# ChuheHong/arm-spmv

Hardware: AMD Instinct MI355X
Metric: SpMV GFLOP/s + achieved HBM GB/s (% roofline), fp64 CSR, 1/2/4/8 MI355X (higher is better)
Workload: dtype f64

## Files before the change

### arm-spmv_amd/csrc/kernels_csr_panel.hip

```cpp
#include <vector>

#include <atomic>

#include "common.hpp"
#include "panel_groups.hpp"
#include "panel_settings.hpp"
#include "wave.hpp"

namespace spmv
{
namespace
{
constexpr int kPanelThreads = 1024;
constexpr int kLineDoubles  = 16;

__global__ __launch_bounds__(256) void panel_count_kernel(const int32_t* __restrict__ gstart, int W, int P,
                                                          const int32_t* __restrict__ row_ptr,
                                                          const int32_t* __restrict__ col,
                                                          int32_t* __restrict__ tile_ptr )
{
    extern __shared__ int32_t hist[];
    const int g  = blockIdx.x;
    const int r0 = gstart[g], r1 = gstart[g + 1];
    for (int i = threadIdx.x; i <= P; i += blockDim.x) hist[i] = 0;
    __syncthreads();
    const int begin = row_ptr[r0], end = row_ptr[r1];
    for (int e = begin + threadIdx.x; e < end; e += blockDim.x) atomicAdd(&hist[col[e] / W], 1);
    __syncthreads();
    if (threadIdx.x < kWave)
    {
        const int lane  = threadIdx.x;
        int       carry = 0;
        for (int base = 0; base < P; base += kWave)
        {
            const int v    = (base + lane < P) ? hist[base + lane] : 0;
            int       incl = v;
            for (int d = 1; d < kWave; d <<= 1)
            {
                const int up = bpermute(incl, max(lane - d, 0));
                if (lane >= d) incl += up;
            }
            if (base + lane < P) tile_ptr[(size_t)g * (P + 1) + base + lane] = carry + incl - v;
            carry += bpermute(incl, kWave - 1);
        }
        if (lane == 0) tile_ptr[(size_t)g * (P + 1) + P] = carry;
    }
}

__global__ __launch_bounds__(256) void panel_scatter_kernel(const int32_t* __restrict__ gstart, int W, int P,
                                                            const int32_t* __restrict__ row_ptr,
                                                            const int32_t* __restrict__ col,
                                                            const double* __restrict__ val,
                                                            const int32_t* __restrict__ tile_ptr,
                                                            int32_t* __restrict__ out_col, uint16_t* __restrict__ out_row,
                                                            double* __restrict__ out_val)
{
    extern __shared__ int32_t cursor[];
    constexpr int LPR = 8;
    const int     g   = blockIdx.x;
    const int     r0 = gstart[g], r1 = gstart[g + 1];
    for (int i = threadIdx.x; i < P; i += blockDim.x) cursor[i] = tile_ptr[(size_t)g * (P + 1) + i];
    __syncthreads();
    const int base = row_ptr[r0];
    for (int r = r0 + threadIdx.x / LPR; r < r1; r += blockDim.x / LPR)
    {
        const int end = row_ptr[r + 1];
        for (int j = row_ptr[r] + threadIdx.x % LPR; j < end; j += LPR)
        {
            const int c   = col[j];
            const int pos = base + atomicAdd(&cursor[c / W], 1);
            out_col[pos]  = c;
            out_row[pos]  = (uint16_t)(r - r0);
            out_val[pos]  = val[j];
        }
    }
}

__global__ __launch_bounds__(256) void panel_line_sort_kernel(int64_t ntiles, const int32_t* __restrict__ gstart, int W, int P,
                                                              const int32_t* __restrict__ row_ptr,
                                                              const int32_t* __restrict__ tile_ptr,
                                                              const int32_t* __restrict__ src_col,
                                                              const uint16_t* __restrict__ src_row,
                                                              const double* __restrict__ src_val,
                                                              int32_t* __restrict__ dst_col, uint16_t* __restrict__ dst_row,
                                                              double* __restrict__ dst_val)
{
    extern __shared__ int32_t bins[];
    const int nb = W / kLineDoubles;
    for (int64_t tile = blockIdx.x; tile < ntiles; tile += gridDim.x)
    {
    const int g    = (int)(tile / P);
    const int p    = (int)(tile % P);
    const int base = row_ptr[gstart[g]];
    const int t0   = base + tile_ptr[(size_t)g * (P + 1) + p];
    const int t1   = base + tile_ptr[(size_t)g * (P + 1) + p + 1];
    if (t0 == t1) continue;
    const int c0 = p * W;
    for (int i = threadIdx.x; i <= nb; i += blockDim.x) bins[i] = 0;
    __syncthreads();
    for (int e = t0 + threadIdx.x; e < t1; e += blockDim.x) atomicAdd(&bins[(src_col[e] - c0) / kLineDoubles], 1);
    __syncthreads();
    if (threadIdx.x < kWave)
    {
        const int lane  = threadIdx.x;
        int       carry = 0;
        for (int b = 0; b < nb; b += kWave)
        {
            const int v    = (b + lane < nb) ? bins[b + lane] : 0;
            int       incl = v;
            for (int d = 1; d < kWave; d <<= 1)
            {
                const int up = bpermute(incl, max(lane - d, 0));
                if (lane >= d) incl += up;
            }
            if (b + lane < nb) bins[b + lane] = carry + incl - v;
            carry += bpermute(incl, kWave - 1);
        }
    }
    __syncthreads();
    for (int e = t0 + threadIdx.x; e < t1; e += blockDim.x)
    {
        const int c   = src_col[e];
        const int pos = t0 + atomicAdd(&bins[(c - c0) / kLineDoubles], 1);
        dst_col[pos]  = c;
        dst_row[pos]  = src_row[e];
        dst_val[pos]  = src_val[e];
    }
    __syncthreads();
    }
}

using u32x2p = unsigned __attribute__((ext_vector_type(2)));

template <int UNROLL, int LAYOUT>
struct PanelBatch
{
    int      c[UNROLL];
    unsigned r[UNROLL];
    double   v[UNROLL];
    __device__ __forceinline__ void unpack(const int32_t* __restrict__ sb, int rowbits)
    {
        if constexpr (LAYOUT >= 3)
        {
#pragma unroll
            for (int u = 0; u < UNROLL; ++u)
            {
                const unsigned w = (unsigned)c[u];
                c[u]             = sb[u] + (int)(w >> rowbits);
                r[u]             = w & ((1u << rowbits) - 1u);
            }
        }
    }
    __device__ __forceinline__ void load(const int32_t* __restrict__ pcol, const uint16_t* __restrict__ prow,
                                         const double* __restrict__ pval, int e, const int32_t* __restrict__ sb = nullptr,
                                         int rowbits = 0)
    {
        load_raw(pcol, prow, pval, e);
        unpack(sb, rowbits);
    }
    __device__ __forceinline__ void load_raw(const int32_t* __restrict__ pcol, const uint16_t* __restrict__ prow,
                                             const double* __restrict__ pval, int e)
    {
        if constexpr (LAYOUT == 4 && UNROLL >= 2)
        {
            const int     t  = e & (kPanelThreads - 1);
            const size_t  p0 = (size_t)(e >> 11) * kPanelThreads + t;
            const u32x2p* w2 = reinterpret_cast<const u32x2p*>(pcol) + p0;
            const f64x2*  v2 = reinterpret_cast<const f64x2*>(pval) + p0;
#pragma unroll
            for (int u = 0; u < UNROLL / 2; ++u)
            {
                const u32x2p w = load_stream(w2 + (size_t)u * kPanelThreads);
                const f64x2  d = load_stream(v2 + (size_t)u * kPanelThreads);
                c[2 * u]       = (int)w.x;
                c[2 * u + 1]   = (int)w.y;
                v[2 * u]       = d.x;
                v[2 * u + 1]   = d.y;
            }
        }
        else if constexpr (LAYOUT == 4)
        {
            const int    t  = e & (kPanelThreads - 1), sl = e >> 10;
            const size_t at = ((size_t)(sl >> 1) << 11) + 2 * (size_t)t + (size_t)(sl & 1);
            c[0]            = load_stream(pcol + at);
            v[0]            = load_stream(pval + at);
        }
        else
        {
#pragma unroll
            for (int u = 0; u < UNROLL; ++u)
            {
                c[u] = load_stream(pcol + e + u * kPanelThreads);
                if constexpr (LAYOUT < 3) r[u] = load_stream(prow + e + u * kPanelThreads);
                v[u] = load_stream(pval + e + u * kPanelThreads);
            }
        }
    }
    __device__ __forceinline__ void apply(const double* __restrict__ x, double* acc) const
    {
        double xv[UNROLL];
        gather(x, xv);
        add(acc, xv);
    }
    __device__ __forceinline__ void gather(const double* __restrict__ x, double (&xv)[UNROLL]) const
    {
#pragma unroll
        for (int u = 0; u < UNROLL; ++u) xv[u] = x[c[u]];
    }
    __device__ __forceinline__ void add(double* acc, const double (&xv)[UNROLL]) const
    {
#pragma unroll
        for (int u = 0; u < UNROLL; ++u) atomicAdd(&acc[r[u]], v[u] * xv[u]);
    }
    __device__ static __forceinline__ void one(const int32_t* __restrict__ pcol, const uint16_t* __restrict__ prow,
                                               const double* __restrict__ pval, int e, const double* __restrict__ x,
                                               double* acc, const int32_t* __restrict__ sb = nullptr, int rowbits = 0)
    {
        PanelBatch<1, LAYOUT> b;
        b.load(pcol, prow, pval, e, sb, rowbits);
        b.apply(x, acc);
    }
};

struct PanelPacked
{
    const int32_t* sbase;
    const int32_t* soff;
    int            rowbits;
};

__global__ void panel_cut_kernel(const int32_t* __restrict__ gstart, int ngroups, const int32_t* __restrict__ row_ptr,
                                 const int32_t* __restrict__ col, int colbits, const int32_t* __restrict__ soff,
                                 int32_t* __restrict__ nslices, int32_t* __restrict__ sbase, int32_t* __restrict__ ssrc,
                                 int32_t* __restrict__ scount)
{
    const int g = blockIdx.x * blockDim.x + threadIdx.x;
    if (g >= ngroups) return;
    const int begin = row_ptr[gstart[g]], end = row_ptr[gstart[g + 1]];
    int       pos = begin, k = 0;
    while (pos < end)
    {
        const int base_line  = col[pos] / kLineDoubles;
        const int limit_line = base_line + (1 << (colbits - 4));
        const int most       = min(kPanelThreads, end - pos);
        int       take       = most;
        if (col[pos + most - 1] / kLineDoubles >= limit_line)
        {
            int lo = 1, hi = most - 1;
            while (lo < hi)
            {
                const int mid = (lo + hi + 1) / 2;
                if (col[pos + mid - 1] / kLineDoubles < limit_line)
                    lo = mid;
                else
                    hi = mid - 1;
            }
            take = lo;
        }
        if (soff)
        {
            const int idx = soff[g] + k;
            sbase[idx]    = base_line * kLineDoubles;
            ssrc[idx]     = pos;
            scount[idx]   = take;
        }
        pos += take;
        ++k;
    }
    if (!soff) nslices[g] = k;
}

__global__ __launch_bounds__(256) void panel_expand_kernel(int total, const int32_t* __restrict__ sbase,
                                                           const int32_t* __restrict__ ssrc,
                                                           const int32_t* __restrict__ scount, const int32_t* __restrict__ col,
                                                           const uint16_t* __restrict__ row, const double* __restrict__ val,
                                                           int rowbits, unsigned pad_row, int pair,
                                                           uint32_t* __restrict__ packed, double* __restrict__ pval)
{
    const unsigned pad = pad_row;
    for (int sl = blockIdx.x; sl < total; sl += gridDim.x)
    {
        const int base = sbase[sl], src = ssrc[sl], cnt = scount[sl];
        for (int j = threadIdx.x; j < kPanelThreads; j += 256)
        {
            const size_t dst = pair ? ((size_t)(sl >> 1) << 11) + 2 * (size_t)j + (size_t)(sl & 1) : (size_t)sl * kPanelThreads + j;
            if (j < cnt)
            {
                packed[dst] = ((unsigned)(col[src + j] - base) << rowbits) | (unsigned)row[src + j];
                pval[dst]   = val[src + j];
            }
            else
            {
                packed[dst] = pad;
                pval[dst]   = 0.0;
            }
        }
    }
}

__global__ void group_nnz_max_kernel(const int32_t* __restrict__ gstart, int ngroups, const int32_t* __restrict__ row_ptr,
                                     int32_t* __restrict__ out_max)
{
    const int g = blockIdx.x * blockDim.x + threadIdx.x;
    if (g >= ngroups) return;
    const int r0 = gstart[g], r1 = gstart[g + 1];
    atomicMax(out_max, row_ptr[r1] - row_ptr[r0]);
}


template <int UNROLL, int LAYOUT, int ORDER, bool TRIAL, int SYNCT>
__global__ __launch_bounds__(kPanelThreads) void csr_panel_pp_kernel(const int32_t* __restrict__ gstart, int ngroups, const int32_t* __restrict__ row_ptr,
                                                                     const int32_t* __restrict__ pcol, const uint16_t* __restrict__ prow,
                                                                     const double* __restrict__ pval, const double* __restrict__ x,
                                                                     double* __restrict__ y, const int32_t* __restrict__ sbase,
                                                                     const int32_t* __restrict__ soff, int rowbits, int overwrite,
                                                                     const double* __restrict__ dot_w, double* __restrict__ dot_out)
{
    extern __shared__ double acc[];
    constexpr int STEP = UNROLL * kPanelThreads;
    const int     lane = threadIdx.x & 63;
    for (int g = blockIdx.x; g < ngroups; g += gridDim.x)
    {
        const int r0   = gstart[g];
        const int rows = gstart[g + 1] - r0;
        for (int i = threadIdx.x; i < rows; i += kPanelThreads) acc[i] = 0.0;
        __syncthreads();
        const int begin = LAYOUT >= 3 ? soff[g] * kPanelThreads : row_ptr[r0];
        const int end   = LAYOUT >= 3 ? soff[g + 1] * kPanelThreads : row_ptr[r0 + rows];
        const int nfull = (end - begin) / STEP;
        const int e0    = begin + threadIdx.x;
        const int32_t* __restrict__ sb = LAYOUT >= 3 ? sbase + soff[g] : pcol;
        PanelBatch<UNROLL, LAYOUT> A, B;
        auto chunk = [&](PanelBatch<UNROLL, LAYOUT>& cur, PanelBatch<UNROLL, LAYOUT>& nxt, int b) __attribute__((always_inline)) {
            if constexpr (SYNCT == 1)
            {
                __syncthreads();
                __builtin_amdgcn_sched_barrier(0);
            }
            const int e_next = e0 + (b + 1 < nfull ? b + 1 : b) * STEP;
            if constexpr (ORDER == 0) cur.load_raw(pcol, prow, pval, e0 + b * STEP);
            if constexpr (ORDER == 1)
            {
                nxt.load_raw(pcol, prow, pval, e_next);
                __builtin_amdgcn_sched_barrier(0);
            }
            cur.unpack(sb + b * UNROLL, rowbits);
            double xv[UNROLL];
            cur.gather(x, xv);
            __builtin_amdgcn_sched_barrier(0);
            if constexpr (ORDER == 2)
            {
                nxt.load_raw(pcol, prow, pval, e_next);
                __builtin_amdgcn_sched_barrier(0);
            }
            if constexpr (SYNCT == 3)
            {
                __syncthreads();
                __builtin_amdgcn_sched_barrier(0);
            }
            cur.add(acc, xv);
            __builtin_amdgcn_sched_barrier(0);
        };
        if (ORDER != 0 && nfull > 0) A.load_raw(pcol, prow, pval, e0);
        int b = 0;
        for (; b + 1 < nfull; b += 2)
        {
            chunk(A, B, b);
            chunk(B, A, b + 1);
        }
        if (b < nfull) chunk(A, B, b);
        int e = e0 + nfull * STEP;
        for (int t = nfull * UNROLL; e < end; e += kPanelThreads, ++t) PanelBatch<1, LAYOUT>::one(pcol, prow, pval, e, x, acc, sb + t, rowbits);
        __syncthreads();
        double part = 0.0;
        for (int i = threadIdx.x; i < rows; i += kPanelThreads)
        {
            const double yn = overwrite ? acc[i] : y[r0 + i] + acc[i];
            y[r0 + i]       = yn;
            if (dot_w) part = fma(dot_w[r0 + i], yn, part);
        }
        if (dot_w)
        {
            part = wave_sum(part);
            if (lane == 0) slot_add(dot_out, part);
        }
        __syncthreads();
    }
}

}

void csr_panel_free(spmv_mat* m)
{
    if (m->pb_col) (void)hipFree(m->pb_col);
    if (m->pb_row) (void)hipFree(m->pb_row);
    if (m->pb_val) (void)hipFree(m->pb_val);
    if (m->pb_pack) (void)hipFree(m->pb_pack);
    if (m->pb_sbase) (void)hipFree(m->pb_sbase);
    if (m->pb_soff) (void)hipFree(m->pb_soff);
    if (m->pb_gstart) (void)hipFree(m->pb_gstart);
    m->pb_gstart = nullptr;
    m->pb_pack   = nullptr;
    m->pb_pair   = false;
    m->pb_sbase  = nullptr;
    m->pb_soff   = nullptr;
    m->pb_col = nullptr;
    m->pb_row = nullptr;
    m->pb_val = nullptr;
    m->pb_built_sort = -1;
    m->pb_tuned_key = 0;
    m->pb_unroll_tuned = 0;
    m->device_bytes -= m->pb_bytes;
    m->pb_bytes = 0;
}

static int pick_group_rows(int nrow, int cap)
{
    for (int m = 1;; ++m)
    {
        const int64_t g = ceil_div(nrow, (int64_t)kNumCu * m);
        if (g <= cap) return (int)std::max<int64_t>(g, 1);
    }
}

static void panel_pack(spmv_mat* m, int ngroups, int max_rows, bool pair)
{
    spmv_ctx*   ctx     = m->ctx;
    hipStream_t s       = ctx->stream;
    const int   rowbits = 32 - __builtin_clz((unsigned)std::max(1, max_rows));
    const int   colbits = 32 - rowbits;
    int32_t *d_n = nullptr, *ssrc = nullptr, *scount = nullptr;
    uint32_t* pack = nullptr;
    double*   pval = nullptr;
    int32_t * sbase = nullptr, *d_soff = nullptr;
    bool      ok   = false;
    do
    {
        if (rowbits > 16 || hipMalloc(&d_n, sizeof(int32_t) * (size_t)ngroups) != hipSuccess) break;
        const unsigned gb = (unsigned)ceil_div(ngroups, 64);
        hipLaunchKernelGGL(panel_cut_kernel, dim3(gb), dim3(64), 0, s, m->pb_gstart, ngroups, m->a, m->pb_col, colbits,
                           (const int32_t*)nullptr, d_n, (int32_t*)nullptr, (int32_t*)nullptr, (int32_t*)nullptr);
        std::vector<int32_t> soff((size_t)ngroups + 1, 0);
        if (hipMemcpyAsync(soff.data() + 1, d_n, sizeof(int32_t) * (size_t)ngroups, hipMemcpyDeviceToHost, s) != hipSuccess ||
            hipStreamSynchronize(s) != hipSuccess)
            break;
        int64_t total = 0;
        for (int g = 1; g <= ngroups; ++g)
        {
            total += pair ? (soff[(size_t)g] + 1) / 2 * 2 : soff[(size_t)g];
            if (total > INT32_MAX / kPanelThreads) break;
            soff[(size_t)g] = (int32_t)total;
        }
        const int64_t padded = total * kPanelThreads;
        if (total > INT32_MAX / kPanelThreads || padded * 12 > m->nnz * 13 + (int64_t)ngroups * kPanelThreads * 12 * (pair ? 2 : 1)) break;
        if (hipMalloc(&ssrc, sizeof(int32_t) * (size_t)total) != hipSuccess ||
            hipMalloc(&scount, sizeof(int32_t) * (size_t)total) != hipSuccess ||
            hipMalloc(&sbase, sizeof(int32_t) * (size_t)total) != hipSuccess ||
            hipMalloc(&d_soff, sizeof(int32_t) * soff.size()) != hipSuccess ||
            hipMalloc(&pack, sizeof(uint32_t) * (size_t)padded) != hipSuccess || hipMalloc(&pval, sizeof(double) * (size_t)padded) != hipSuccess)
            break;
        if (hipMemcpyAsync(d_soff, soff.data(), sizeof(int32_t) * soff.size(), hipMemcpyHostToDevice, s) != hipSuccess) break;
        if (hipMemsetAsync(sbase, 0, sizeof(int32_t) * (size_t)total, s) != hipSuccess || hipMemsetAsync(ssrc, 0, sizeof(int32_t) * (size_t)total, s) != hipSuccess ||
            hipMemsetAsync(scount, 0, sizeof(int32_t) * (size_t)total, s) != hipSuccess)
            break;
        hipLaunchKernelGGL(panel_cut_kernel, dim3(gb), dim3(64), 0, s, m->pb_gstart, ngroups, m->a, m->pb_col, colbits,
                           (const int32_t*)d_soff, (int32_t*)nullptr, sbase, ssrc, scount);
        hipLaunchKernelGGL(panel_expand_kernel, dim3((unsigned)std::min<int64_t>(total, kMaxGrid * 4)), dim3(256), 0, s,
                           (int)total, sbase, ssrc, scount, m->pb_col, m->pb_row, m->pb_val, rowbits, (unsigned)max_rows, pair ? 1 : 0, pack,
                           pval);
        if (hipGetLastError() != hipSuccess || hipStreamSynchronize(s) != hipSuccess) break;
        ok = true;
        (void)hipFree(m->pb_col);
        (void)hipFree(m->pb_row);
        (void)hipFree(m->pb_val);
        m->pb_col     = nullptr;
        m->pb_row     = nullptr;
        m->pb_val     = pval;
        m->pb_pack    = pack;
        m->pb_sbase   = sbase;
        m->pb_soff    = d_soff;
        m->pb_rowbits = rowbits;
        m->pb_pair    = pair;
        m->pb_slices  = (int32_t)total;
        m->pb_bytes   = padded * 12 + (int64_t)sizeof(int32_t) * (total + ngroups + 1);
    } while (0);
    if (d_n) (void)hipFree(d_n);
    if (ssrc) (void)hipFree(ssrc);
    if (scount) (void)hipFree(scount);
    if (!ok)
    {
        if (pack) (void)hipFree(pack);
        if (pval) (void)hipFree(pval);
        if (sbase) (void)hipFree(sbase);
        if (d_soff) (void)hipFree(d_soff);
        (void)hipGetLastError();
    }
}

int csr_panel_build(spmv_mat* m)
{
    spmv_ctx* ctx = m->ctx;
    if (m->nrow == 0 || m->nnz == 0) return SPMV_OK;
    constexpr int kCapRows = 20000;
    int G = m->pb_group_rows > 0 ? std::min(m->pb_group_rows, kCapRows) : pick_group_rows(m->nrow, kCapRows);
    G     = std::max<int64_t>(G, ceil_div(m->nrow, (int64_t)1 << 21));
    int W = m->pb_panel_width > 0 ? m->pb_panel_width : 128 * 1024;
    W     = std::min(524288, std::max(kLineDoubles, (W / kLineDoubles) * kLineDoubles));
    while (ceil_div(m->ncol, W) > 8192) W *= 2;
    const bool sort = m->pb_sort != 0;
    const bool pack = (m->pb_aos == 3 || m->pb_aos == 4) && sort;
    if (m->pb_val && m->pb_built_rows == G && m->pb_built_width == W && m->pb_built_sort == (int)sort && m->pb_built_layout == m->pb_aos &&
        (m->pb_rounds_req == 0 || m->pb_rounds_req == m->pb_built_rounds))
        return panel_choose_pace(m);
    if (!m->b || !m->v) SPMV_FAIL(SPMV_ERR_INVALID, "the panel layout cannot be re-built: this handle gave up its CSR arrays (panel_keep_csr = 0)");
    csr_panel_free(m);
    std::vector<int32_t> gstart;
    int                  try_rounds = 0;
    {
        std::vector<int32_t> rp((size_t)m->nrow + 1);
        SPMV_HIP(hipMemcpyAsync(rp.data(), m->a, sizeof(int32_t) * rp.size(), hipMemcpyDeviceToHost, ctx->stream));
        SPMV_HIP(hipStreamSynchronize(ctx->stream));
        const int want = (int)ceil_div(m->nrow, G);
        if (m->pb_group_rows > 0)
            (void)panel_cut(rp, m->nrow, (int64_t)INT32_MAX, G, &gstart);
        else
        {
            const double busiest = panel_balanced_cut(rp, m->nrow, want, kCapRows, kNumCu, &gstart);
            if (m->pb_rounds_req > 1)
                (void)panel_balanced_cut(rp, m->nrow, want * m->pb_rounds_req, kCapRows, kNumCu, &gstart);
            else if (m->pb_rounds_req == 0 && select_trials_enabled(m))
                try_rounds = panel_rounds_worth_a_trial(rp, m->nrow, want, kCapRows, kNumCu, busiest);
        }
    }
    const int ngroups = (int)gstart.size() - 1;
    int       max_rows = 0;
    for (int g = 0; g < ngroups; ++g) max_rows = std::max(max_rows, gstart[(size_t)g + 1] - gstart[(size_t)g]);
    SPMV_HIP(hipMalloc(&m->pb_gstart, sizeof(int32_t) * gstart.size()));
    SPMV_HIP(hipMemcpyAsync(m->pb_gstart, gstart.data(), sizeof(int32_t) * gstart.size(), hipMemcpyHostToDevice, ctx->stream));
    SPMV_HIP(hipStreamSynchronize(ctx->stream));
    const int P       = (int)ceil_div(m->ncol, W);
    const size_t nnz  = (size_t)m->nnz;

    int32_t*  tile_ptr = nullptr;
    int32_t*  tcol     = nullptr;
    uint16_t* trow     = nullptr;
    double*   tval     = nullptr;
    int       rc       = SPMV_OK;
    hipStream_t s      = ctx->stream;
    do
    {
        if (hipMalloc(&m->pb_col, nnz * sizeof(int32_t)) != hipSuccess || hipMalloc(&m->pb_row, nnz * sizeof(uint16_t)) != hipSuccess ||
            hipMalloc(&m->pb_val, nnz * sizeof(double)) != hipSuccess ||
            hipMalloc(&tile_ptr, sizeof(int32_t) * (size_t)ngroups * (P + 1)) != hipSuccess)
        {
            rc = SPMV_ERR_ALLOC;
            break;
        }
        if (sort && (hipMalloc(&tcol, nnz * sizeof(int32_t)) != hipSuccess || hipMalloc(&trow, nnz * sizeof(uint16_t)) != hipSuccess ||
                     hipMalloc(&tval, nnz * sizeof(double)) != hipSuccess))
        {
            rc = SPMV_ERR_ALLOC;
            break;
        }
        hipLaunchKernelGGL(panel_count_kernel, dim3(ngroups), dim3(256), sizeof(int32_t) * (P + 1), s, m->pb_gstart, W, P,
                           m->a, m->b, tile_ptr);
        int32_t*  scol = sort ? tcol : m->pb_col;
        uint16_t* srow = sort ? trow : m->pb_row;
        double*   sval = sort ? tval : m->pb_val;
        hipLaunchKernelGGL(panel_scatter_kernel, dim3(ngroups), dim3(256), sizeof(int32_t) * P, s, m->pb_gstart, W, P, m->a,
                           m->b, m->v, tile_ptr, scol, srow, sval);
        if (sort && sizeof(int32_t) * (W / kLineDoubles + 1) > 65536)
            (void)hipFuncSetAttribute((const void*)panel_line_sort_kernel, hipFuncAttributeMaxDynamicSharedMemorySize, 160008);
        if (sort)
            hipLaunchKernelGGL(panel_line_sort_kernel, dim3((unsigned)std::min<int64_t>((int64_t)ngroups * P, (int64_t)1 << 22)), dim3(256),
                               sizeof(int32_t) * (W / kLineDoubles + 1), s, (int64_t)ngroups * P, m->pb_gstart, W, P, m->a, tile_ptr, tcol, trow,
                               tval, m->pb_col, m->pb_row, m->pb_val);
        if (hipGetLastError() != hipSuccess || hipStreamSynchronize(s) != hipSuccess) rc = SPMV_ERR_HIP;
    } while (0);
    if (tile_ptr) (void)hipFree(tile_ptr);
    if (tcol) (void)hipFree(tcol);
    if (trow) (void)hipFree(trow);
    if (tval) (void)hipFree(tval);
    if (rc != SPMV_OK)
    {
        csr_panel_free(m);
        SPMV_FAIL(rc, "building the panel layout (%d groups of %d rows, %d panels of %d columns) failed: %s", ngroups, G, P,
                  W, hipGetErrorString(hipGetLastError()));
    }
    m->pb_built_rows  = G;
    m->pb_max_rows    = max_rows;
    m->pb_built_width = W;
    m->pb_built_sort  = (int)sort;
    m->pb_ngroups     = ngroups;
    {
        SPMV_TRY(ensure_scratch(ctx, 64));
        int32_t* d_max = (int32_t*)ctx->scratch;
        int32_t  h_max = 0;
        SPMV_HIP(hipMemsetAsync(d_max, 0, sizeof(int32_t), s));
        hipLaunchKernelGGL(group_nnz_max_kernel, dim3((unsigned)ceil_div(ngroups, 256)), dim3(256), 0, s, m->pb_gstart, ngroups,
                           m->a, d_max);
        SPMV_HIP(hipMemcpyAsync(&h_max, d_max, sizeof(int32_t), hipMemcpyDeviceToHost, s));
        SPMV_HIP(hipStreamSynchronize(s));
        m->pb_max_group_nnz = h_max;
    }
    m->pb_bytes       = (int64_t)(nnz * 14);
    m->pb_built_layout = m->pb_aos;
    if (pack) panel_pack(m, ngroups, max_rows, m->pb_aos == 4);
    m->device_bytes += m->pb_bytes;
    m->pb_built_rounds = m->pb_rounds_req > 1 ? m->pb_rounds_req : 1;
    SPMV_TRY(panel_choose_pace(m));
    if (try_rounds > 1)
    {
        select_scratch sv;
        if (sv.alloc(ctx, m->ncol, m->nrow) != SPMV_OK) return SPMV_OK;
        float t_one = 0.f, t_more = 0.f;
        int   rc    = select_time(ctx, [&] { return csr_panel_apply(ctx, m, sv.x, sv.y); }, 1e30f, &t_one);
        if (rc != SPMV_OK) return rc;
        m->pb_rounds_req = try_rounds;
        if ((rc = csr_panel_build(m)) != SPMV_OK)
        {
            (void)hipGetLastError();
            m->pb_rounds_req = 1;
            rc               = csr_panel_build(m);
            m->pb_rounds_req = 0;
            return rc;
        }
        rc = select_time(ctx, [&] { return csr_panel_apply(ctx, m, sv.x, sv.y); }, 1e30f, &t_more);
        if (rc == SPMV_OK && !(t_more < 0.97f * t_one))
        {
            m->pb_rounds_req = 1;
            rc               = csr_panel_build(m);
        }
        m->pb_rounds_req = 0;
        m->pb_rounds_us[0] = t_one * 1000.f;
        m->pb_rounds_us[1] = t_more * 1000.f;
        return rc;
    }
    return SPMV_OK;
}

static int panel_launch(spmv_ctx* ctx, const spmv_mat* A, const double* x, double* y, bool trial, const apply_extra& ex);

int panel_choose_pace(spmv_mat* m)
{
    spmv_ctx* ctx = m->ctx;
    const int key = 1000 + std::max(m->pb_unroll, 0) * 10 + (m->pb_pipe + 1) + ((m->pb_sync + 1) & 7) * 1000000;
    if (m->pb_tuned_key == key) return SPMV_OK;
    m->pb_tuned_key    = 0;
    m->pb_unroll_tuned = 0;
    m->pb_pipe_tuned   = 0;
    m->pb_sync_tuned   = 0;
    if (m->pb_unroll > 0 && m->pb_pipe >= 0 && m->pb_sync >= 0) return SPMV_OK;
    const bool worth = (double)m->ncol * 8.0 > 4.0 * 1048576.0 && m->pb_max_group_nnz >= 8LL * 8 * kPanelThreads;
    if (!worth) return SPMV_OK;
    if (!select_trials_enabled(m))
    {
        m->pb_unroll_tuned = m->pb_unroll <= 0 ? 8 : 0;
        m->pb_pipe_tuned   = m->pb_pack ? 2 : 1;
        m->pb_sync_tuned   = 1;
        m->pb_tuned_key    = key;
        return SPMV_OK;
    }
    select_scratch sv;
    if (sv.alloc(ctx, m->ncol, m->nrow) != SPMV_OK) return SPMV_OK;
    double *x = sv.x, *y = sv.y;
    int  rc    = SPMV_OK;
    auto launch = [&] { return panel_launch(ctx, m, x, y, true, apply_extra{}); };
    auto timed  = [&](int launches, float* ms) -> int {
        SPMV_TRY(launch());
        return time_launches(ctx, launches, launch, ms);
    };
    struct Try
    {
        int unroll, pipe, sync;
    };
    const Try packed_tries[] = {{8, 2, 1}, {8, 2, 3}, {4, 2, 3}, {8, 1, 1}, {8, 1, 3}, {4, 2, 1}, {4, 1, 0}, {8, 1, 0}};
    const Try plain_tries[]  = {{8, 1, 1}, {4, 1, 1}, {4, 1, 3}, {8, 2, 1}, {8, 1, 0}, {4, 1, 0}, {2, 1, 0}};
    const Try* tries  = m->pb_pack ? packed_tries : plain_tries;
    const int  ntries = m->pb_pack ? 8 : 7;
    Try    best{m->pb_unroll > 0 ? m->pb_unroll : 8, m->pb_pipe >= 0 ? m->pb_pipe : 1, m->pb_sync >= 0 ? m->pb_sync : 0};
    double best_ms = 1e30;
    int    tried   = 0;
    for (int pass = 0; pass < 2 && rc == SPMV_OK; ++pass)
    {
        for (int i = 0; i < (pass == 0 ? ntries : 1) && rc == SPMV_OK; ++i)
        {
            const Try t = pass == 0 ? tries[i] : best;
            if (pass == 0 && ((m->pb_unroll > 0 && m->pb_unroll != t.unroll) || (m->pb_pipe >= 0 && m->pb_pipe != t.pipe) ||
                              (m->pb_sync >= 0 && m->pb_sync != t.sync)))
                continue;
            if (pass == 1 && tried > 0) break;
            m->pb_unroll_tuned = t.unroll;
            m->pb_pipe_tuned   = t.pipe;
            m->pb_sync_tuned   = t.sync;
            float a = 0.f, b = 0.f;
            if ((rc = timed(4, &a)) != SPMV_OK || (rc = timed(4, &b)) != SPMV_OK) break;
            ++tried;
            const double ms = std::min(a, b);
            if (ms < best_ms * (best_ms < 1e29 ? 0.99 : 1.0))
            {
                best_ms = ms;
                best    = t;
            }
        }
    }
    (void)hipStreamSynchronize(ctx->stream);
    sv.release();
    m->pb_unroll_tuned = rc == SPMV_OK && m->pb_unroll <= 0 ? best.unroll : 0;
    m->pb_pipe_tuned   = rc == SPMV_OK ? best.pipe : 0;
    m->pb_sync_tuned   = rc == SPMV_OK ? best.sync : 0;
    m->pb_tuned_key    = rc == SPMV_OK ? key : 0;
    return rc;
}

int csr_panel_apply(spmv_ctx* ctx, const spmv_mat* A, const double* x, double* y)
{
    return panel_launch(ctx, A, x, y, false, apply_extra{});
}
int csr_panel_apply_ex(spmv_ctx* ctx, const spmv_mat* A, const double* x, double* y, const apply_extra& ex)
{
    return panel_launch(ctx, A, x, y, false, ex);
}

static int panel_launch(spmv_ctx* ctx, const spmv_mat* A, const double* x, double* y, bool trial, const apply_extra& ex)
{
    if (A->nrow == 0 || A->nnz == 0)
    {
        if (ex.overwrite && A->nrow > 0) SPMV_TRY(vec_fill(ctx, y, A->nrow, 0.0));
        return SPMV_OK;
    }
    if (!A->pb_val) SPMV_FAIL(SPMV_ERR_INVALID, "panel kernel selected but its layout was not built");
    const size_t lds = ((size_t)A->pb_max_rows + (A->pb_pack ? 1 : 0)) * sizeof(double);
    const int per_cu = (lds <= 80000 && A->pb_two_per_cu) ? 2 : 1;
    const int grid   = std::min(A->pb_ngroups, kNumCu * per_cu);
    const panel_settings run = panel_effective(A->pb_unroll, A->pb_unroll_tuned, A->pb_pipe, A->pb_pipe_tuned, A->pb_sync, A->pb_sync_tuned);
    const int unroll = run.unroll, pipe = run.pipe, sync = run.sync;
    const int layout = A->pb_pack ? (A->pb_pair ? 4 : 3) : 0;
    const bool have = layout >= 3 ? (A->pb_pack && A->pb_sbase && A->pb_soff && A->pb_val && A->pb_rowbits > 0 && A->pb_rowbits < 32)
                                  : (A->pb_col && A->pb_row && A->pb_val);
    if (!A->pb_gstart || !x || !y || !have)
        SPMV_FAIL(SPMV_ERR_INVALID, "panel kernel: layout %d is selected but its arrays are not there", layout);
    const int32_t* arg_col = layout >= 3 ? (const int32_t*)A->pb_pack : A->pb_col;
#define SPMV_PANEL_PP(U, LY, OR, TR, SY)                                                                                               \
    {                                                                                                                                  \
        static std::atomic<unsigned long long> granted{0};                                                         \
        if (!((granted.load(std::memory_order_relaxed) >> ctx->device) & 1ull))                                                        \
        {                                                                                                                              \
            SPMV_HIP(hipFuncSetAttribute((const void*)csr_panel_pp_kernel<U, LY, OR, TR, SY>, hipFuncAttributeMaxDynamicSharedMemorySize, 160008)); \
            granted.fetch_or(1ull << ctx->device, std::memory_order_relaxed);                                                          \
        }                                                                                                                              \
        hipLaunchKernelGGL((csr_panel_pp_kernel<U, LY, OR, TR, SY>), dim3(grid), dim3(kPanelThreads), lds, ctx->stream, A->pb_gstart,  \
                           A->pb_ngroups, A->a, arg_col, A->pb_row, A->pb_val, x, y, A->pb_sbase, A->pb_soff, A->pb_rowbits,           \
                           ex.overwrite ? 1 : 0, ex.dot_w, ex.dot_out);                                                                \
        SPMV_HIP(hipGetLastError());                                                                                                   \
        return SPMV_OK;                                                                                                                \
    }
#define SPMV_PANEL_PP_SY(U, LY, OR)                                                                        \
    if (unroll == U && layout == LY && pipe == OR)                                                         \
    {                                                                                                      \
        if (sync == 0) { if (trial) SPMV_PANEL_PP(U, LY, OR, true, 0) SPMV_PANEL_PP(U, LY, OR, false, 0) } \
        if (sync == 1) { if (trial) SPMV_PANEL_PP(U, LY, OR, true, 1) SPMV_PANEL_PP(U, LY, OR, false, 1) } \
        if (sync == 3) { if (trial) SPMV_PANEL_PP(U, LY, OR, true, 3) SPMV_PANEL_PP(U, LY, OR, false, 3) } \
    }
#define SPMV_PANEL_PP_OR(U, LY) SPMV_PANEL_PP_SY(U, LY, 0) SPMV_PANEL_PP_SY(U, LY, 1) SPMV_PANEL_PP_SY(U, LY, 2)
    SPMV_PANEL_PP_OR(8, 4) SPMV_PANEL_PP_OR(4, 4) SPMV_PANEL_PP_OR(2, 4)
    SPMV_PANEL_PP_OR(8, 3) SPMV_PANEL_PP_OR(4, 3) SPMV_PANEL_PP_OR(2, 3)
    SPMV_PANEL_PP_OR(8, 0) SPMV_PANEL_PP_OR(4, 0) SPMV_PANEL_PP_OR(2, 0)
#undef SPMV_PANEL_PP_OR
#undef SPMV_PANEL_PP_SY
#undef SPMV_PANEL_PP
    SPMV_FAIL(SPMV_ERR_INVALID, "panel kernel: unroll=%d layout=%d order=%d sync=%d is not instantiated", unroll, layout, pipe, sync);
}
}
```

Baseline: 576.4.

## Prefetch panel row bases, batch the tail, and hoist LDS accumulator zeroing

New measurement: 581.5 (median of 6 runs). About the same (+0.9%).

```diff
diff --git a/arm-spmv_amd/csrc/kernels_csr_panel.hip b/arm-spmv_amd/csrc/kernels_csr_panel.hip
--- a/arm-spmv_amd/csrc/kernels_csr_panel.hip
+++ b/arm-spmv_amd/csrc/kernels_csr_panel.hip
@@ -1,6 +1,7 @@
 #include <vector>
 
 #include <atomic>
+#include <type_traits>
 
 #include "common.hpp"
 #include "panel_groups.hpp"
@@ -314,27 +315,38 @@
                                                                      const double* __restrict__ pval, const double* __restrict__ x,
                                                                      double* __restrict__ y, const int32_t* __restrict__ sbase,
                                                                      const int32_t* __restrict__ soff, int rowbits, int overwrite,
-                                                                     const double* __restrict__ dot_w, double* __restrict__ dot_out)
+                                                                     const double* __restrict__ dot_w, double* __restrict__ dot_out, int nacc)
 {
     extern __shared__ double acc[];
     constexpr int STEP = UNROLL * kPanelThreads;
     const int     lane = threadIdx.x & 63;
+    for (int i = threadIdx.x; i < nacc; i += kPanelThreads) acc[i] = 0.0;
+    __syncthreads();
     for (int g = blockIdx.x; g < ngroups; g += gridDim.x)
     {
         const int r0   = gstart[g];
         const int rows = gstart[g + 1] - r0;
-        for (int i = threadIdx.x; i < rows; i += kPanelThreads) acc[i] = 0.0;
-        __syncthreads();
         const int begin = LAYOUT >= 3 ? soff[g] * kPanelThreads : row_ptr[r0];
         const int end   = LAYOUT >= 3 ? soff[g + 1] * kPanelThreads : row_ptr[r0 + rows];
         const int nfull = (end - begin) / STEP;
         const int e0    = begin + threadIdx.x;
         const int32_t* __restrict__ sb = LAYOUT >= 3 ? sbase + soff[g] : pcol;
         PanelBatch<UNROLL, LAYOUT> A, B;
-        auto chunk = [&](PanelBatch<UNROLL, LAYOUT>& cur, PanelBatch<UNROLL, LAYOUT>& nxt, int b) __attribute__((always_inline)) {
+        int32_t bases[LAYOUT >= 3 ? 2 * UNROLL : 1] = {};
+        auto load_bases = [&](int32_t (&to)[LAYOUT >= 3 ? 2 * UNROLL : 1], int pair) __attribute__((always_inline)) {
+            if constexpr (LAYOUT >= 3)
+            {
+#pragma unroll
+                for (int u = 0; u < 2 * UNROLL; ++u) to[u] = sb[pair * UNROLL + u];
+                __builtin_amdgcn_sched_barrier(0);
+                __builtin_amdgcn_s_waitcnt(0xC07F);
+                __builtin_amdgcn_sched_barrier(0);
+            }
+        };
+        auto chunk = [&](PanelBatch<UNROLL, LAYOUT>& cur, PanelBatch<UNROLL, LAYOUT>& nxt, int b, const int32_t* cb, auto fetch, int next_pair) __attribute__((always_inline)) {
             if constexpr (SYNCT == 1)
             {
-                __syncthreads();
+                __builtin_amdgcn_s_barrier();
                 __builtin_amdgcn_sched_barrier(0);
             }
             const int e_next = e0 + (b + 1 < nfull ? b + 1 : b) * STEP;
@@ -344,7 +356,7 @@
                 nxt.load_raw(pcol, prow, pval, e_next);
                 __builtin_amdgcn_sched_barrier(0);
             }
-            cur.unpack(sb + b * UNROLL, rowbits);
+            cur.unpack(cb, rowbits);
             double xv[UNROLL];
             cur.gather(x, xv);
             __builtin_amdgcn_sched_barrier(0);
@@ -358,24 +370,45 @@
                 __syncthreads();
                 __builtin_amdgcn_sched_barrier(0);
             }
+            if constexpr (decltype(fetch)::value) load_bases(bases, next_pair);
             cur.add(acc, xv);
             __builtin_amdgcn_sched_barrier(0);
         };
         if (ORDER != 0 && nfull > 0) A.load_raw(pcol, prow, pval, e0);
+        if (nfull > 1) load_bases(bases, 0);
         int b = 0;
         for (; b + 1 < nfull; b += 2)
         {
-            chunk(A, B, b);
-            chunk(B, A, b + 1);
-        }
-        if (b < nfull) chunk(A, B, b);
+            chunk(A, B, b, bases, std::false_type{}, 0);
+            chunk(B, A, b + 1, bases + (LAYOUT >= 3 ? UNROLL : 0), std::true_type{}, min(b + 2, nfull - 2));
+        }
+        if (b < nfull) chunk(A, B, b, sb + b * UNROLL, std::false_type{}, 0);
         int e = e0 + nfull * STEP;
-        for (int t = nfull * UNROLL; e < end; e += kPanelThreads, ++t) PanelBatch<1, LAYOUT>::one(pcol, prow, pval, e, x, acc, sb + t, rowbits);
+        int t = nfull * UNROLL;
+        const int left = (end - begin) / kPanelThreads - t;
+        auto batch = [&](auto n) __attribute__((always_inline)) {
+            constexpr int N = decltype(n)::value;
+            if (left & N)
+            {
+                PanelBatch<N, LAYOUT> T;
+                T.load(pcol, prow, pval, e, sb + t, rowbits);
+                T.apply(x, acc);
+                e += N * kPanelThreads;
+                t += N;
+            }
+        };
+        if constexpr (UNROLL > 4) batch(std::integral_constant<int, 4>{});
+        if constexpr (UNROLL > 2) batch(std::integral_constant<int, 2>{});
+        batch(std::integral_constant<int, 1>{});
+        if constexpr (LAYOUT < 3)
+            if (e < end) PanelBatch<1, LAYOUT>::one(pcol, prow, pval, e, x, acc);
         __syncthreads();
         double part = 0.0;
         for (int i = threadIdx.x; i < rows; i += kPanelThreads)
         {
-            const double yn = overwrite ? acc[i] : y[r0 + i] + acc[i];
+            const double a  = acc[i];
+            acc[i]          = 0.0;
+            const double yn = overwrite ? a : y[r0 + i] + a;
             y[r0 + i]       = yn;
             if (dot_w) part = fma(dot_w[r0 + i], yn, part);
         }
@@ -751,7 +784,7 @@
         }                                                                                                                              \
         hipLaunchKernelGGL((csr_panel_pp_kernel<U, LY, OR, TR, SY>), dim3(grid), dim3(kPanelThreads), lds, ctx->stream, A->pb_gstart,  \
                            A->pb_ngroups, A->a, arg_col, A->pb_row, A->pb_val, x, y, A->pb_sbase, A->pb_soff, A->pb_rowbits,           \
-                           ex.overwrite ? 1 : 0, ex.dot_w, ex.dot_out);                                                                \
+                           ex.overwrite ? 1 : 0, ex.dot_w, ex.dot_out, (int)(lds / sizeof(double)));                                   \
         SPMV_HIP(hipGetLastError());                                                                                                   \
         return SPMV_OK;                                                                                                                \
     }
```
